# apple/ml-gmpi

Measured on AMD Instinct MI355X. Metric: Mpix*planes/s, higher is better.
Workload: dtype f32; 1 GPU; FFHQ1024-shaped: 1024x1024, 96 planes, batch 4 views, bf16 storage; views_per_gpu=4, views_total=4, H=1024, W=1024, planes=96, variant=auto, strict_order=False, outputs=rgb+depth, parallelism=views sharded x1, poses=truncated-gaussian draw (seed 3) on every rank

## Files before the change

ml-gmpi_amd/csrc/render_band.hip:

```cpp
#include "gmpi_device.hpp"

#include <algorithm>
#include <cstdlib>
#include <type_traits>


namespace gmpi {
namespace band {

constexpr int kNT = 1024;
constexpr int SBW = 64, SBH = 8;
constexpr float kBoxEps = 1.0f / 64;
constexpr int kWindowCols16 = 2, kWindowCols32 = 2, kWindowCols32Deep = 2, kDeepPlanes = 128;
constexpr int kViewRotation = 1;
constexpr int kRunPieces = 2;
constexpr int kTicketTail = 16;
constexpr float kCoordLimit = 16384.0f;

typedef uint32_t u32x4 __attribute__((ext_vector_type(4)));
template <int V> using ic = std::integral_constant<int, V>;

template <int D0, int STEP>
__device__ __forceinline__ void dma16x2(uint32_t voff, uint32_t soff1, const u32x4& rsrc, uint32_t lds_dst, uint64_t m0, uint64_t m1);

#ifndef GMPI_BAND_PPT16
#define GMPI_BAND_PPT16 2
#endif
#ifndef GMPI_BAND_PPT32
#define GMPI_BAND_PPT32 2
#endif
template <typename TexT> struct Geo {
    static constexpr int kES = static_cast<int>(sizeof(TexT));
    static constexpr int NSB = kES == 2 ? 4 : 2;
    static constexpr int PPT = kES == 2 ? GMPI_BAND_PPT16 : GMPI_BAND_PPT32;
    static constexpr int WPS = SBH / PPT;
    static constexpr int kSubLanes = 64 * WPS;
    static constexpr int kThreads = NSB * kSubLanes;
    static constexpr int kWavesPerSimd = kThreads / 128;
    static_assert(kThreads <= kNT && SBH % PPT == 0, "waves");
    static constexpr int kTPI = 16 / kES;
    static constexpr int kCols = kES == 2 ? 10 : 20;
    static constexpr int kLineBytes = kCols * 16;
    static constexpr int kRowBytes = 4 * kLineBytes;
    static constexpr int kIPR = 4 * kCols;
    static constexpr int kMaxRows = 15;
    static constexpr int kCapItems = kMaxRows * kIPR;
    static constexpr int kSubBytes = kCapItems * 16;
    static constexpr int kBufBytes = NSB * kSubBytes;
    static constexpr int kRPP = kSubLanes / kIPR;
    static constexpr int kPassItems = kRPP * kIPR;
    static constexpr int kNP = (kMaxRows + kRPP - 1) / kRPP;
    static_assert(kNP == 3 || kNP == 5, "passes");
    static constexpr int kOffBytes = kThreads * 4;
    static constexpr int kLdsBytes = kOffBytes + 2 * kBufBytes;
};
static_assert(Geo<bf16_t>::kLdsBytes * 2 <= 160 * 1024 && Geo<f16_t>::kLdsBytes * 2 <= 160 * 1024 && Geo<float>::kLdsBytes * 2 <= 160 * 1024, "2 workgroups per CU");

__device__ __forceinline__ void dma16(uint32_t voff, uint32_t soff, const u32x4& rsrc, uint32_t lds_dst, uint64_t mask) {
    uint64_t save;
    asm volatile("s_mov_b64 %0, exec\n\ts_mov_b64 exec, %4\n\ts_mov_b32 m0, %3\n\ts_nop 0\n\tbuffer_load_dwordx4 %1, %2, %5 offen lds\n\ts_mov_b64 exec, %0"
                 : "=&s"(save) : "v"(voff), "s"(rsrc), "s"(lds_dst), "s"(mask), "s"(soff) : "memory");
}
template <int D0, int STEP>
__device__ __forceinline__ void dma16x3(uint32_t voff, uint32_t soff1, uint32_t soff2, const u32x4& rsrc, uint32_t lds_dst, uint64_t m0, uint64_t m1, uint64_t m2) {
    uint64_t save;
    asm volatile("s_mov_b64 %0, exec\n\t"
                 "s_mov_b64 exec, %4\n\ts_add_i32 m0, %3, %9\n\ts_nop 0\n\tbuffer_load_dwordx4 %1, %2, 0 offen lds\n\t"
                 "s_mov_b64 exec, %5\n\ts_add_i32 m0, %3, %10\n\ts_nop 0\n\tbuffer_load_dwordx4 %1, %2, %7 offen lds\n\t"
                 "s_mov_b64 exec, %6\n\ts_add_i32 m0, %3, %11\n\ts_nop 0\n\tbuffer_load_dwordx4 %1, %2, %8 offen lds\n\t"
                 "s_mov_b64 exec, %0"
                 : "=&s"(save) : "v"(voff), "s"(rsrc), "s"(lds_dst), "s"(m0), "s"(m1), "s"(m2), "s"(soff1), "s"(soff2), "i"(D0), "i"(D0 + STEP), "i"(D0 + 2 * STEP)
                 : "memory", "scc");
}
template <int D0, int STEP>
__device__ __forceinline__ void dma16x2(uint32_t voff, uint32_t soff1, const u32x4& rsrc, uint32_t lds_dst, uint64_t m0, uint64_t m1) {
    uint64_t save;
    asm volatile("s_mov_b64 %0, exec\n\t"
                 "s_mov_b64 exec, %4\n\ts_add_i32 m0, %3, %7\n\ts_nop 0\n\tbuffer_load_dwordx4 %1, %2, 0 offen lds\n\t"
                 "s_mov_b64 exec, %5\n\ts_add_i32 m0, %3, %8\n\ts_nop 0\n\tbuffer_load_dwordx4 %1, %2, %6 offen lds\n\t"
                 "s_mov_b64 exec, %0"
                 : "=&s"(save) : "v"(voff), "s"(rsrc), "s"(lds_dst), "s"(m0), "s"(m1), "s"(soff1), "i"(D0), "i"(D0 + STEP)
                 : "memory", "scc");
}
template <int D0, int STEP>
__device__ __forceinline__ void dma16x4(uint32_t voff, uint32_t s1, uint32_t s2, uint32_t s3, const u32x4& rsrc, uint32_t lds_dst, uint64_t m0, uint64_t m1, uint64_t m2, uint64_t m3) {
    uint64_t save;
    asm volatile("s_mov_b64 %0, exec\n\t"
                 "s_mov_b64 exec, %4\n\ts_add_i32 m0, %3, %11\n\ts_nop 0\n\tbuffer_load_dwordx4 %1, %2, 0 offen lds\n\t"
                 "s_mov_b64 exec, %5\n\ts_add_i32 m0, %3, %12\n\ts_nop 0\n\tbuffer_load_dwordx4 %1, %2, %8 offen lds\n\t"
                 "s_mov_b64 exec, %6\n\ts_add_i32 m0, %3, %13\n\ts_nop 0\n\tbuffer_load_dwordx4 %1, %2, %9 offen lds\n\t"
                 "s_mov_b64 exec, %7\n\ts_add_i32 m0, %3, %14\n\ts_nop 0\n\tbuffer_load_dwordx4 %1, %2, %10 offen lds\n\t"
                 "s_mov_b64 exec, %0"
                 : "=&s"(save) : "v"(voff), "s"(rsrc), "s"(lds_dst), "s"(m0), "s"(m1), "s"(m2), "s"(m3), "s"(s1), "s"(s2), "s"(s3),
                   "i"(D0), "i"(D0 + STEP), "i"(D0 + 2 * STEP), "i"(D0 + 3 * STEP)
                 : "memory", "scc");
}
template <int D0, int STEP>
__device__ __forceinline__ void dma16x5(uint32_t voff, uint32_t s1, uint32_t s2, uint32_t s3, uint32_t s4, const u32x4& rsrc, uint32_t lds_dst, uint64_t m0, uint64_t m1, uint64_t m2,
                                        uint64_t m3, uint64_t m4) {
    uint64_t save;
    asm volatile("s_mov_b64 %0, exec\n\t"
                 "s_mov_b64 exec, %4\n\ts_add_i32 m0, %3, %13\n\ts_nop 0\n\tbuffer_load_dwordx4 %1, %2, 0 offen lds\n\t"
                 "s_mov_b64 exec, %5\n\ts_add_i32 m0, %3, %14\n\ts_nop 0\n\tbuffer_load_dwordx4 %1, %2, %9 offen lds\n\t"
                 "s_mov_b64 exec, %6\n\ts_add_i32 m0, %3, %15\n\ts_nop 0\n\tbuffer_load_dwordx4 %1, %2, %10 offen lds\n\t"
                 "s_mov_b64 exec, %7\n\ts_add_i32 m0, %3, %16\n\ts_nop 0\n\tbuffer_load_dwordx4 %1, %2, %11 offen lds\n\t"
                 "s_mov_b64 exec, %8\n\ts_add_i32 m0, %3, %17\n\ts_nop 0\n\tbuffer_load_dwordx4 %1, %2, %12 offen lds\n\t"
                 "s_mov_b64 exec, %0"
                 : "=&s"(save) : "v"(voff), "s"(rsrc), "s"(lds_dst), "s"(m0), "s"(m1), "s"(m2), "s"(m3), "s"(m4), "s"(s1), "s"(s2), "s"(s3), "s"(s4),
                   "i"(D0), "i"(D0 + STEP), "i"(D0 + 2 * STEP), "i"(D0 + 3 * STEP), "i"(D0 + 4 * STEP)
                 : "memory", "scc");
}
__device__ __forceinline__ void wg_barrier() { asm volatile("s_waitcnt vmcnt(0) lgkmcnt(0)\n\ts_barrier" ::: "memory"); }
template <int O> __device__ __forceinline__ void tap16(uint32_t& t, uint32_t a) {
    asm volatile("ds_read_u16_d16_hi %0, %1 offset:%2" : "=v"(t) : "v"(a), "i"(O));
}
template <int O> __device__ __forceinline__ void tap32x2(uint32_t& t0, uint32_t& t1, uint32_t a) {
    typedef uint32_t u32x2 __attribute__((ext_vector_type(2)));
    u32x2 v;
    asm volatile("ds_read2_b32 %0, %1 offset0:%2 offset1:%3" : "=v"(v) : "v"(a), "i"(O), "i"(O + 1));
    t0 = v.x, t1 = v.y;
}

__device__ __forceinline__ void band_pos(int brem, int bands_x, int bands_y, int wc, int& bxi, int& byi) {
    const int per_window = wc * bands_y;
    const int g = brem / per_window, r = brem - g * per_window;
    const int cols = min(wc, bands_x - g * wc);
    byi = r / cols;
    bxi = g * wc + (r - byi * cols);
}

constexpr int kPlU4 = 2;
__device__ __forceinline__ uint32_t shape_pack(int nq, int rows, int clo, int ncol, int rlo, int nrow, bool inside) {
    return inside ? static_cast<uint32_t>(nq | rows << 5)
                  : static_cast<uint32_t>(nq | rows << 5 | clo << 9 | ncol << 14 | rlo << 19 | nrow << 23) | 0x80000000u;
}
struct Shape { int nq, rows; uint32_t clo, ncol, rlo, nrow; };
__device__ __forceinline__ Shape shape_unpack(uint32_t w) {
    Shape h;
    h.nq = w & 31, h.rows = (w >> 5) & 15;
    const bool padded = (w >> 31) != 0;
    h.clo = padded ? (w >> 9) & 31 : 0u, h.ncol = padded ? (w >> 14) & 31 : static_cast<uint32_t>(h.nq);
    h.rlo = padded ? (w >> 19) & 15 : 0u, h.nrow = padded ? (w >> 23) & 15 : static_cast<uint32_t>(h.rows);
    return h;
}
template <typename TexT, bool AC>
__global__ __launch_bounds__(1024) void band_table_kernel(const KParams p, const int bands_x, const int bands_y, const int n_bands, const float cx, const float cy,
                                                         uint4* __restrict__ recs, uint4* __restrict__ pl, uint32_t* __restrict__ hdr, uint32_t* __restrict__ tickets) {
    using G = Geo<TexT>;
    constexpr int kES = G::kES, kTPI = G::kTPI, kCols = G::kCols, kMaxRows = G::kMaxRows, kRowBytes = G::kRowBytes, kSubBytes = G::kSubBytes;
    constexpr int NSB = G::NSB;
    static_assert(kCols < 32 && kMaxRows < 16, "shape_pack");
    const int band_id = blockIdx.x;
    int n, brem;
    item_to_view(p, band_id, bands_x * bands_y, n, brem);
    int bxi, byi;
    band_pos(brem, bands_x, bands_y, p.band_cols, bxi, byi);
    uint32_t ignore = 0;
    const int m = view_mpi(p, n, ignore);
    const int Ht = p.Ht, Wt = p.Wt, H = p.H, W = p.W;
    const float ex = p.eye_pos[3 * n + 0], ey = p.eye_pos[3 * n + 1], ez = p.eye_pos[3 * n + 2];
    const int64_t HW = static_cast<int64_t>(H) * W;
    const float* __restrict__ rdv = p.ray_dir + static_cast<int64_t>(n) * 3 * HW;
    const TexT* __restrict__ vol = static_cast<const TexT*>(p.rgba) + static_cast<int64_t>(m) * p.s_mpi;
    const int sx0 = min(bxi * (NSB * SBW), W - 1), sy0 = byi * SBH;
    const int by0p = min(sy0, H - 1), by1p = min(sy0 + SBH - 1, H - 1);
    bool unfit = false;
    for (int i = threadIdx.x; i < p.D * NSB; i += blockDim.x) {
        const int b = i % NSB, k = i / NSB;
        const float* __restrict__ dhw = p.dhw + (static_cast<int64_t>(m) * p.D + k) * 3;
        const float d = dhw[0], ph = dhw[1], pw = dhw[2];
        const float zdiff = d - ez;
        const float hw = pw * 0.5f, hh = ph * 0.5f;
        const int bx0p = min(sx0 + b * SBW, W - 1), bx1p = min(sx0 + b * SBW + SBW - 1, W - 1);
        float mnx = __builtin_inff(), mxx = -__builtin_inff(), mny = mnx, mxy = mxx;
        bool finite = true;
        const float rw_a = __builtin_amdgcn_rcpf(hw), rh_a = __builtin_amdgcn_rcpf(hh);
#pragma unroll
        for (int c = 0; c < 4; ++c) {
            const int64_t q = static_cast<int64_t>((c & 2) ? by1p : by0p) * W + ((c & 1) ? bx1p : bx0p);
            float ix, iy, sc;
            const float crz = rdv[2 * HW + q];
            plane_coord_recip<AC>(zdiff, hw, hh, rw_a, rh_a, ex, ey, rdv[q], rdv[HW + q], crz, __builtin_amdgcn_rcpf(crz), cx, cy, ix, iy, sc);
            finite = finite && (fabsf(ix) < kCoordLimit) && (fabsf(iy) < kCoordLimit);
            mnx = fminf(mnx, ix), mxx = fmaxf(mxx, ix), mny = fminf(mny, iy), mxy = fmaxf(mxy, iy);
        }
        int qx0 = 0, by0 = 0, nq = -1, nrows = 0;
        if (finite) {
            const int bx0 = static_cast<int>(floorf(mnx - kBoxEps)), bx1 = static_cast<int>(floorf(mxx + kBoxEps)) + 1;
            by0 = static_cast<int>(floorf(mny - kBoxEps));
            const int by1 = static_cast<int>(floorf(mxy + kBoxEps)) + 1;
            qx0 = bx0 & ~(kTPI - 1);
            nq = (bx1 - qx0) / kTPI + 1;
            nrows = by1 - by0 + 1;
            if (nq > kCols || nrows > kMaxRows) nq = -1;
        }
        uint32_t shape = 0;
        if (nq > 0) {
            const int clo = min(max(-qx0 / kTPI, 0), nq), chi = min(max((Wt - qx0) / kTPI, 0), nq);
            const int rlo = min(max(-by0, 0), nrows), rhi = min(max(Ht - by0, 0), nrows);
            const bool inside = clo == 0 && chi == nq && rlo == 0 && rhi == nrows;
            shape = shape_pack(nq, nrows, clo, chi - clo, rlo, rhi - rlo, inside);
        } else {
            qx0 = 0, by0 = 0;
            unfit = true;
        }
        const uint64_t origin = reinterpret_cast<uint64_t>(vol + (static_cast<int64_t>(k) * p.s_plane + static_cast<int64_t>(by0) * p.s_row + qx0));
        const int gpart = b * kSubBytes - (by0 * kRowBytes + qx0 * kES);
        recs[(static_cast<int64_t>(band_id) * p.D + k) * NSB + b] =
            make_uint4(static_cast<uint32_t>(origin & 0xffffffffu), static_cast<uint32_t>((origin >> 32) & 0xffffu), shape, static_cast<uint32_t>(gpart));
        if (brem == 0 && b == 0) {
            uint4* r = pl + (static_cast<int64_t>(n) * p.D + k) * kPlU4;
            r[0] = make_uint4(__float_as_uint(zdiff), __float_as_uint(hw), __float_as_uint(hh), __float_as_uint(1.0f / hw));
            r[1] = make_uint4(__float_as_uint(1.0f / hh), 0u, 0u, 0u);
        }
    }
    if (blockIdx.x == 0 && threadIdx.x < 8) tickets[threadIdx.x] = 0u;
    const int any_unfit = __syncthreads_or(unfit ? 1 : 0);
    if (threadIdx.x == 0) {
        hdr[band_id] = static_cast<uint32_t>(any_unfit);
        if (any_unfit && p.gate != nullptr) {
            if (p.view_to_mpi == nullptr && p.views_per_mpi > 1) {
                const int first = n / p.views_per_mpi * p.views_per_mpi, size = min(p.views_per_mpi, p.N - first);
                for (int v = 0; v < size; ++v) p.gate[first + v] = p.gate_gen;
            } else {
                p.gate[n] = p.gate_gen;
            }
        }
    }
}

template <typename TexT, bool AC, bool STRICT, bool CHECK>
__global__ __launch_bounds__(Geo<TexT>::kThreads, Geo<TexT>::kWavesPerSimd) void render_band_kernel(const KParams p, const int bands_x, const int bands_y, const int n_bands, const float cx, const float cy,
                                                         const uint4* __restrict__ recs, const uint4* __restrict__ pl, const uint32_t* __restrict__ hdr, uint32_t* __restrict__ tickets) {
    using G = Geo<TexT>;
    constexpr int kES = G::kES, kTPI = G::kTPI, kCols = G::kCols, kNP = G::kNP;
    constexpr int NSB = G::NSB, PPT = G::PPT, WPS = G::WPS, kSubLanes = G::kSubLanes;
    constexpr int kLineBytes = G::kLineBytes, kRowBytes = G::kRowBytes, kSubBytes = G::kSubBytes, kBufBytes = G::kBufBytes;
    constexpr int kRPP = G::kRPP, kPassItems = G::kPassItems;
    constexpr bool BF = kES == 2;
    constexpr bool F16 = std::is_same<TexT, f16_t>::value;

    __shared__ __attribute__((aligned(16))) unsigned char smem[G::kLdsBytes];
    typedef __attribute__((address_space(3))) unsigned char lds_byte;
    const uint32_t tile_base = static_cast<uint32_t>(reinterpret_cast<uintptr_t>((lds_byte*)smem));

    const int group_items = bands_x * bands_y * (p.view_to_mpi == nullptr ? p.views_per_mpi : 1);
    int band_id;
    {
        const int per_xcd = (group_items + 7) / 8, n_groups = (n_bands + group_items - 1) / group_items, static_blocks = per_xcd * 8 * n_groups;
        const int T = min(p.band_tail, per_xcd);
        const int jb = static_cast<int>(blockIdx.x) / 8, x = static_cast<int>(blockIdx.x) % 8;
        const bool ticketed = T > 0 && (static_cast<int>(blockIdx.x) >= static_blocks || (jb / per_xcd == n_groups - 1 && jb % per_xcd >= per_xcd - T));
        if (!ticketed) {
            band_id = blockIdx.x < static_cast<unsigned>(static_blocks) ? xcd_item_per_group(blockIdx.x, group_items, n_bands, p.band_rot, p.band_split) : n_bands;
        } else {
            int* word = reinterpret_cast<int*>(smem + 2 * kBufBytes);
            if (threadIdx.x == 0) {
                int got = n_bands;
                for (int i = 0; i < 8; ++i) {
                    const int q = (x + i) % 8;
                    const int t = static_cast<int>(atomicAdd(tickets + q, 1u));
                    if (t < T) {
                        got = xcd_item_per_group(q + 8 * ((n_groups - 1) * per_xcd + per_xcd - T + t), group_items, n_bands, p.band_rot, p.band_split);
                        break;
                    }
                }
                *word = got;
            }
            __syncthreads();
            band_id = __builtin_amdgcn_readfirstlane(*word);
            __syncthreads();
        }
    }
// ... 30 lines not shown
    const int64_t s_chan = p.s_chan, s_row = p.s_row;

    check_camera_behind(p, vw, brem == 0 && tid == 0);

    const int px = bxi * (NSB * SBW) + sb * SBW + lane;
    const int py0 = byi * SBH + wj;
    const int pxc = min(px, W - 1);
    float rx[PPT], ry[PPT], rz[PPT], rcp_rz[PPT];
    Accum A[PPT];
#pragma unroll
    for (int q = 0; q < PPT; ++q) {
        const int64_t pix = static_cast<int64_t>(min(py0 + WPS * q, H - 1)) * W + pxc;
        rx[q] = rdv[pix], ry[q] = rdv[HW + pix], rz[q] = rdv[2 * HW + pix];
        rcp_rz[q] = 1.0f / rz[q];
    }
    auto ray_dot = [&](int q) { return gmpi::ray_dot(vw, rx[q], ry[q], rz[q]); };

    auto loader_pos = [&](int& l_col, int& l_line, int& l_row, bool& l_on) {
        const int t = fresh_tid() & (kSubLanes - 1);
        l_line = t / kCols, l_col = t - l_line * kCols, l_row = l_line >> 2, l_on = t < kPassItems;
    };
    {
        int l_col, l_line, l_row;
        bool l_on;
        loader_pos(l_col, l_line, l_row, l_on);
        reinterpret_cast<uint32_t*>(smem + 2 * kBufBytes)[tid] = static_cast<uint32_t>(l_row * s_row + (l_line & 3) * s_chan + kTPI * l_col) * static_cast<uint32_t>(kES);
    }
    const uint32_t pass_off = static_cast<uint32_t>(kRPP * s_row) * static_cast<uint32_t>(kES), pass_off2 = 2 * pass_off;
    const uint32_t pass_off3 = 3 * pass_off, pass_off4 = 4 * pass_off;
    const uint32_t sub_base = tile_base + static_cast<uint32_t>(sb * kSubBytes);
    const uint32_t wave_dst = sub_base + static_cast<uint32_t>(wj) * 1024u;

#ifdef GMPI_TUNE
    const bool abl_noload = (p.flags & (1u << 16)) != 0, abl_nocomp = (p.flags & (1u << 17)) != 0, abl_noissue = (p.flags & (1u << 18)) != 0;
    const bool abl_nobar = (p.flags & (1u << 20)) != 0, abl_norec = (p.flags & (1u << 21)) != 0;
#else
    constexpr bool abl_noload = false, abl_nocomp = false, abl_noissue = false, abl_nobar = false, abl_norec = false;
#endif

#ifdef GMPI_PROF
    uint32_t prof_acc[8] = {0, 0, 0, 0, 0, 0, 0, 0};
    uint64_t prof_last, prof_start;
    asm volatile("s_memtime %0\n\ts_waitcnt lgkmcnt(0)" : "=s"(prof_start));
    prof_last = prof_start;
#define GMPI_STAMP(i) do { uint64_t now_; asm volatile("s_memtime %0\n\ts_waitcnt lgkmcnt(0)" : "=s"(now_)); prof_acc[i] += static_cast<uint32_t>(now_ - prof_last); prof_last = now_; } while (0)
#else
#define GMPI_STAMP(i) do { } while (0)
#endif

    const uint4* __restrict__ myrec = recs + (static_cast<int64_t>(band_id) * D * NSB + sb);
    const uint4* __restrict__ mypl = pl + static_cast<int64_t>(n) * D * kPlU4;
    constexpr int kRecStep = NSB;

    if (hdr[band_id] != 0) {
#pragma unroll
        for (int q = 0; q < PPT; ++q) {
            const float dot = ray_dot(q);
            for (int t = 0; t < D; ++t) {
                uint32_t gbad = 0;
                gather_plane<TexT, AC, STRICT>(p, vw, vol, t, dhw[3 * t] - ez, dhw[3 * t + 1], dhw[3 * t + 2], rx[q], ry[q], rz[q], dot, std::bool_constant<CHECK>{}, gbad, A[q]);
                if (check_range && __any(gbad != 0)) bad_w |= GMPI_STATUS_RGBA_RANGE;
            }
        }
    } else {
        float dots[PPT];
#pragma unroll
        for (int q = 0; q < PPT; ++q) dots[q] = STRICT ? ray_dot(q) : 0.0f;
        uint64_t m_cur[kNP];
        int dims_cur = 0;
        bool three = false;
        int np_cur = kNP - 1;
#pragma unroll
        for (int r = 0; r < kNP; ++r) m_cur[r] = 0;

        auto issue = [&](const uint4& rl, uint32_t g_off, auto ub) {
            constexpr int U = decltype(ub)::value;
            const int dims = static_cast<int>(rl.z);
            const u32x4 rsrc = {static_cast<uint32_t>(__builtin_amdgcn_readfirstlane(static_cast<int>(rl.x))),
                                static_cast<uint32_t>(__builtin_amdgcn_readfirstlane(static_cast<int>(rl.y))), 0x80000000u, 0x00020000u};
            if (dims >= 0) {
                if (dims != dims_cur) {
                    const int nq = dims & 31, rows = dims >> 5;
                    dims_cur = dims;
                    three = rows > (kNP - 1) * kRPP;
                    np_cur = max((rows + kRPP - 1) / kRPP, 3);
                    int l_col, l_line, l_row;
                    bool l_on;
                    loader_pos(l_col, l_line, l_row, l_on);
#pragma unroll
                    for (int r = 0; r < kNP; ++r) {
                        m_cur[r] = __ballot(l_on && l_col < nq && l_row + r * kRPP < rows);
                        if (abl_noload) m_cur[r] = 0;
                    }
                }
                if constexpr (kNP == 3) {
                    if (three) dma16x3<U * kBufBytes, kPassItems * 16>(g_off, pass_off, pass_off2, rsrc, wave_dst, m_cur[0], m_cur[1], m_cur[2]);
                    else dma16x2<U * kBufBytes, kPassItems * 16>(g_off, pass_off, rsrc, wave_dst, m_cur[0], m_cur[1]);
                } else {
                    if (np_cur == 5) dma16x5<U * kBufBytes, kPassItems * 16>(g_off, pass_off, pass_off2, pass_off3, pass_off4, rsrc, wave_dst, m_cur[0], m_cur[1], m_cur[2], m_cur[3], m_cur[4]);
                    else if (np_cur == 4) dma16x4<U * kBufBytes, kPassItems * 16>(g_off, pass_off, pass_off2, pass_off3, rsrc, wave_dst, m_cur[0], m_cur[1], m_cur[2], m_cur[3]);
                    else dma16x3<U * kBufBytes, kPassItems * 16>(g_off, pass_off, pass_off2, rsrc, wave_dst, m_cur[0], m_cur[1], m_cur[2]);
                }
            } else {
                const Shape h = shape_unpack(static_cast<uint32_t>(dims));
                const int rows = h.rows;
                const uint32_t clo = h.clo, ncol = h.ncol, llo = 4 * h.rlo, nline = 4 * h.nrow;
                dims_cur = dims;
                three = rows > (kNP - 1) * kRPP;
                const int npk = (rows + kRPP - 1) / kRPP;
                np_cur = max(npk, 3);
                int l_col, l_line, l_row;
                bool l_on;
                loader_pos(l_col, l_line, l_row, l_on);
#pragma unroll
                for (int r = 0; r < kNP; ++r) {
                    m_cur[r] = __ballot(l_on && l_row + r * kRPP < rows);
                    if (abl_noload) m_cur[r] = 0;
                    if (r < npk) {
                        const bool ok = (static_cast<uint32_t>(l_col) - clo < ncol) & (static_cast<uint32_t>(l_line + 4 * r * kRPP) - llo < nline);
                        dma16(ok ? g_off : 0x80000000u, r * pass_off, rsrc, wave_dst + static_cast<uint32_t>(U * kBufBytes + r * (kPassItems * 16)), m_cur[r]);
                    }
                }
            }
        };

        uint32_t chk_acc = 0;
        auto tap_fold8 = [&](const uint32_t (&q)[8]) {
            asm volatile("v_max3_u32 %0, %0, %1, %2\n\tv_max3_u32 %0, %0, %3, %4\n\tv_max3_u32 %0, %0, %5, %6\n\tv_max3_u32 %0, %0, %7, %8"
                         : "+v"(chk_acc) : "v"(q[0]), "v"(q[1]), "v"(q[2]), "v"(q[3]), "v"(q[4]), "v"(q[5]), "v"(q[6]), "v"(q[7]));
        };

        auto tapf = [&](uint32_t t) -> float {
            if constexpr (F16) {
                typedef _Float16 h2_t __attribute__((ext_vector_type(2)));
                return static_cast<float>(__builtin_bit_cast(h2_t, t).y);
            } else {
                return __uint_as_float(t);
            }
        };
        struct Coords { float s, nw, ne, sw, se; uint32_t a_tap; };
        auto coords = [&](int q, const float4& rf, const float2& rg, Coords& c) {
            float ix, iy, fx, fy;
            if (STRICT) {
                float u, v;
                plane_coord<AC>(rf.x, rf.z + rf.z, rf.y + rf.y, ex, ey, rx[q], ry[q], rz[q], cx, cy, ix, iy, c.s, u, v);
                fx = floorf(ix), fy = floorf(iy);
                const float fx1 = fx + 1.0f, fy1 = fy + 1.0f;
                const float wx1 = ix - fx, wx0 = fx1 - ix, wy1 = iy - fy, wy0 = fy1 - iy;
                c.nw = wx0 * wy0, c.ne = wx1 * wy0, c.sw = wx0 * wy1, c.se = wx1 * wy1;
            } else {
                plane_coord_recip<AC>(rf.x, rf.y, rf.z, rf.w, rg.x, ex, ey, rx[q], ry[q], rz[q], rcp_rz[q], cx, cy, ix, iy, c.s);
                fx = floorf(ix), fy = floorf(iy);
                const float wx1 = ix - fx, wy1 = iy - fy;
                const float wx0 = 1.0f - wx1, wy0 = 1.0f - wy1;
                c.nw = wx0 * wy0, c.ne = wx1 * wy0, c.sw = wx0 * wy1, c.se = wx1 * wy1;
            }
            const float af = __builtin_fmaf(fy, static_cast<float>(kRowBytes), __builtin_fmaf(fx, static_cast<float>(kES), rg.y));
            c.a_tap = static_cast<uint32_t>(static_cast<int32_t>(af));
        };
        auto taps = [&](auto hb, uint32_t a_tap, uint32_t (&q)[8]) {
            constexpr int C0 = 2 * decltype(hb)::value;
            if constexpr (BF) {
                asm volatile("ds_read_u16_d16_hi %0, %8 offset:%9\n\tds_read_u16_d16_hi %1, %8 offset:%10\n\tds_read_u16_d16_hi %2, %8 offset:%11\n\tds_read_u16_d16_hi %3, %8 offset:%12\n\t"
                             "ds_read_u16_d16_hi %4, %8 offset:%13\n\tds_read_u16_d16_hi %5, %8 offset:%14\n\tds_read_u16_d16_hi %6, %8 offset:%15\n\tds_read_u16_d16_hi %7, %8 offset:%16\n\t"
                             "s_waitcnt lgkmcnt(0)"
                             : "=&v"(q[0]), "=&v"(q[1]), "=&v"(q[2]), "=&v"(q[3]), "=&v"(q[4]), "=&v"(q[5]), "=&v"(q[6]), "=&v"(q[7])
                             : "v"(a_tap), "i"(C0 * kLineBytes), "i"(C0 * kLineBytes + 2), "i"(C0 * kLineBytes + kRowBytes), "i"(C0 * kLineBytes + kRowBytes + 2),
                               "i"((C0 + 1) * kLineBytes), "i"((C0 + 1) * kLineBytes + 2), "i"((C0 + 1) * kLineBytes + kRowBytes), "i"((C0 + 1) * kLineBytes + kRowBytes + 2));
            } else {
                typedef uint32_t u32x2 __attribute__((ext_vector_type(2)));
                u32x2 v0, v1, v2, v3;
// ... 11 lines not shown
                         "ds_read_u16_d16_hi %4, %8 offset:%13\n\tds_read_u16_d16_hi %5, %8 offset:%14\n\tds_read_u16_d16_hi %6, %8 offset:%15\n\tds_read_u16_d16_hi %7, %8 offset:%16"
                         : "=&v"(q[0]), "=&v"(q[1]), "=&v"(q[2]), "=&v"(q[3]), "=&v"(q[4]), "=&v"(q[5]), "=&v"(q[6]), "=&v"(q[7])
                         : "v"(a_tap), "i"(C0 * kLineBytes), "i"(C0 * kLineBytes + 2), "i"(C0 * kLineBytes + kRowBytes), "i"(C0 * kLineBytes + kRowBytes + 2),
                           "i"((C0 + 1) * kLineBytes), "i"((C0 + 1) * kLineBytes + 2), "i"((C0 + 1) * kLineBytes + kRowBytes), "i"((C0 + 1) * kLineBytes + kRowBytes + 2));
        };
        auto taps_land = [&](auto nb, uint32_t (&q)[8]) {
            constexpr int N = decltype(nb)::value;
            asm volatile("s_waitcnt lgkmcnt(%8)" : "+v"(q[0]), "+v"(q[1]), "+v"(q[2]), "+v"(q[3]), "+v"(q[4]), "+v"(q[5]), "+v"(q[6]), "+v"(q[7]) : "i"(N));
        };
        typedef uint32_t u32x2_t __attribute__((ext_vector_type(2)));
        auto taps32_issue = [&](auto hb, uint32_t a_tap, uint32_t a_bot, u32x2_t (&v)[4]) {
            constexpr int C0 = 2 * decltype(hb)::value;
            asm volatile("ds_read2_b32 %0, %4 offset0:%6 offset1:%7\n\tds_read2_b32 %1, %5 offset0:%6 offset1:%7\n\t"
                         "ds_read2_b32 %2, %4 offset0:%8 offset1:%9\n\tds_read2_b32 %3, %5 offset0:%8 offset1:%9"
                         : "=&v"(v[0]), "=&v"(v[1]), "=&v"(v[2]), "=&v"(v[3])
                         : "v"(a_tap), "v"(a_bot), "i"(C0 * (kLineBytes / 4)), "i"(C0 * (kLineBytes / 4) + 1), "i"((C0 + 1) * (kLineBytes / 4)), "i"((C0 + 1) * (kLineBytes / 4) + 1));
        };
        auto taps32_land = [&](auto nb, u32x2_t (&v)[4]) {
            constexpr int N = decltype(nb)::value;
            asm volatile("s_waitcnt lgkmcnt(%4)" : "+v"(v[0]), "+v"(v[1]), "+v"(v[2]), "+v"(v[3]) : "i"(N));
        };
        auto pixel = [&](int q, const float4& rf, const float2& rg) {
            Coords c;
            coords(q, rf, rg, c);
            Footprint f;
            f.nw = c.nw, f.ne = c.ne, f.sw = c.sw, f.se = c.se;
            uint32_t t[8];
            float smp[4];
            taps(ic<0>{}, c.a_tap, t);
            if (check_range) tap_fold8(t);
            smp[0] = bilerp<STRICT>(tapf(t[0]), tapf(t[1]), tapf(t[2]), tapf(t[3]), f);
            smp[1] = bilerp<STRICT>(tapf(t[4]), tapf(t[5]), tapf(t[6]), tapf(t[7]), f);
            taps(ic<1>{}, c.a_tap, t);
            if (check_range) tap_fold8(t);
            smp[2] = bilerp<STRICT>(tapf(t[0]), tapf(t[1]), tapf(t[2]), tapf(t[3]), f);
            smp[3] = bilerp<STRICT>(tapf(t[4]), tapf(t[5]), tapf(t[6]), tapf(t[7]), f);
            blend<STRICT>(A[q], smp[0], smp[1], smp[2], smp[3], c.s, dots[q]);
        };


        uint4 Ln, Fc;
        uint32_t rhh_c, gp_c;
        uint32_t g_off = 0;
#ifdef GMPI_PROF
        constexpr bool piped = false, pipedG = false;
#else
        constexpr bool piped = BF && !STRICT && PPT == 2 && kNP == 3;
        constexpr bool pipedG = !STRICT && !piped;
#endif
        auto stage = [&](int tt, auto ub) {
            constexpr int U = decltype(ub)::value;
            if (!abl_nobar) wg_barrier();
            GMPI_STAMP(0);
            if (tt + 1 < D && !abl_noissue) issue(Ln, g_off, ic<1 - U>{});
            GMPI_STAMP(3);
            const float4 rf = make_float4(__uint_as_float(Fc.x), __uint_as_float(Fc.y), __uint_as_float(Fc.z), __uint_as_float(Fc.w));
            const float2 rg = make_float2(__uint_as_float(rhh_c), static_cast<float>(static_cast<int>(gp_c) + static_cast<int>(tile_base) + U * kBufBytes));
            if constexpr (piped) {
                if (!abl_nocomp) {
                    uint32_t ta[8], tb[8];
                    Coords p0, p1;
                    Footprint f;
                    float smp[4];
                    coords(0, rf, rg, p0);
                    taps_issue(ic<0>{}, p0.a_tap, ta);
                    taps_issue(ic<1>{}, p0.a_tap, tb);
                    coords(1, rf, rg, p1);
                    asm volatile("" : "+v"(p1.s), "+v"(p1.nw), "+v"(p1.ne), "+v"(p1.sw), "+v"(p1.se), "+v"(p1.a_tap));
                    taps_land(ic<8>{}, ta);
                    if (check_range) tap_fold8(ta);
                    f.nw = p0.nw, f.ne = p0.ne, f.sw = p0.sw, f.se = p0.se;
                    smp[0] = bilerp<false>(tapf(ta[0]), tapf(ta[1]), tapf(ta[2]), tapf(ta[3]), f);
                    smp[1] = bilerp<false>(tapf(ta[4]), tapf(ta[5]), tapf(ta[6]), tapf(ta[7]), f);
                    asm volatile("" : "+v"(smp[0]), "+v"(smp[1]));
                    taps_issue(ic<0>{}, p1.a_tap, ta);
                    taps_land(ic<8>{}, tb);
                    if (check_range) tap_fold8(tb);
                    smp[2] = bilerp<false>(tapf(tb[0]), tapf(tb[1]), tapf(tb[2]), tapf(tb[3]), f);
                    smp[3] = bilerp<false>(tapf(tb[4]), tapf(tb[5]), tapf(tb[6]), tapf(tb[7]), f);
                    blend<false>(A[0], smp[0], smp[1], smp[2], smp[3], p0.s, dots[0]);
                    asm volatile("" : "+v"(A[0].T), "+v"(A[0].r), "+v"(A[0].g), "+v"(A[0].b), "+v"(A[0].z));
                    taps_issue(ic<1>{}, p1.a_tap, tb);
                    taps_land(ic<8>{}, ta);
                    if (check_range) tap_fold8(ta);
                    f.nw = p1.nw, f.ne = p1.ne, f.sw = p1.sw, f.se = p1.se;
                    smp[0] = bilerp<false>(tapf(ta[0]), tapf(ta[1]), tapf(ta[2]), tapf(ta[3]), f);
                    smp[1] = bilerp<false>(tapf(ta[4]), tapf(ta[5]), tapf(ta[6]), tapf(ta[7]), f);
                    asm volatile("" : "+v"(smp[0]), "+v"(smp[1]));
                    taps_land(ic<0>{}, tb);
                    if (check_range) tap_fold8(tb);
                    smp[2] = bilerp<false>(tapf(tb[0]), tapf(tb[1]), tapf(tb[2]), tapf(tb[3]), f);
                    smp[3] = bilerp<false>(tapf(tb[4]), tapf(tb[5]), tapf(tb[6]), tapf(tb[7]), f);
                    blend<false>(A[1], smp[0], smp[1], smp[2], smp[3], p1.s, dots[1]);
                }
            } else if constexpr (pipedG) {
                constexpr int NB = BF ? 8 : 4;
                if (!abl_nocomp) {
                    uint32_t ta[8], tb[8];
                    u32x2_t va[4], vb[4];
                    Coords pc, pn;
                    Footprint f;
                    float smp[4];
                    auto issueA = [&](const Coords& c) {
                        if constexpr (BF) taps_issue(ic<0>{}, c.a_tap, ta);
                        else taps32_issue(ic<0>{}, c.a_tap, c.a_tap + kRowBytes, va);
                    };
                    auto issueB = [&](const Coords& c) {
// ... 26 lines not shown
                            smp[2] = bilerp<false>(__uint_as_float(vb[0].x), __uint_as_float(vb[0].y), __uint_as_float(vb[1].x), __uint_as_float(vb[1].y), f);
                            smp[3] = bilerp<false>(__uint_as_float(vb[2].x), __uint_as_float(vb[2].y), __uint_as_float(vb[3].x), __uint_as_float(vb[3].y), f);
                        }
                    };
                    auto px_step = [&](auto qc) {
                        constexpr int Q = decltype(qc)::value;
                        constexpr bool more = Q + 1 < PPT;
                        if constexpr (more) {
                            coords(Q + 1, rf, rg, pn);
                            asm volatile("" : "+v"(pn.s), "+v"(pn.nw), "+v"(pn.ne), "+v"(pn.sw), "+v"(pn.se), "+v"(pn.a_tap));
                        }
                        f.nw = pc.nw, f.ne = pc.ne, f.sw = pc.sw, f.se = pc.se;
                        landA(ic<NB>{});
                        if constexpr (more) issueA(pn);
                        landB(ic<(more ? NB : 0)>{});
                        blend<false>(A[Q], smp[0], smp[1], smp[2], smp[3], pc.s, dots[Q]);
                        if constexpr (more) {
                            asm volatile("" : "+v"(A[Q].T), "+v"(A[Q].r), "+v"(A[Q].g), "+v"(A[Q].b), "+v"(A[Q].z));
                            issueB(pn);
                            pc = pn;
                        }
                    };
                    coords(0, rf, rg, pc);
                    issueA(pc);
                    issueB(pc);
                    px_step(ic<0>{});
                    if constexpr (PPT > 1) px_step(ic<1>{});
                    if constexpr (PPT > 2) px_step(ic<2>{});
                    if constexpr (PPT > 3) px_step(ic<3>{});
                    static_assert(PPT <= 4, "pixel slots");
                }
            } else {
                GMPI_STAMP(2);
                if (!abl_nocomp) {
#pragma unroll
                    for (int q = 0; q < PPT; ++q) {
                        pixel(q, rf, rg);
                        GMPI_STAMP(5 + q);
                    }
                }
            }
            if (!abl_norec) {
                gp_c = Ln.w;
                Ln = myrec[static_cast<int64_t>(tt + 2) * kRecStep];
                Fc = mypl[(tt + 1) * kPlU4], rhh_c = mypl[(tt + 1) * kPlU4 + 1].x;
            }
            static_assert(PPT <= 4 && kNP <= 5, "pixel slots / check passes");
        };
#pragma unroll
        for (int q = 0; q < PPT; ++q)
            asm volatile("" : "+v"(rx[q]), "+v"(ry[q]), "+v"(rz[q]), "+v"(rcp_rz[q]), "+v"(A[q].T), "+v"(A[q].r), "+v"(A[q].g), "+v"(A[q].b), "+v"(A[q].z));
        __syncthreads();
        g_off = reinterpret_cast<const uint32_t*>(smem + 2 * kBufBytes)[fresh_tid()];
        issue(myrec[0], g_off, ic<0>{});
        Fc = mypl[0], rhh_c = mypl[1].x, gp_c = myrec[0].w, Ln = myrec[kRecStep];
        for (int t = 0; t < D; t += 2) {
            stage(t, ic<0>{});
            if (t + 1 < D) stage(t + 1, ic<1>{});
        }
        if (check_range) {
            constexpr uint32_t kOne = F16 ? 0x3c00u : BF ? 0x3f80u : 0x3f800000u, kNegZero = BF ? 0x8000u : 0x80000000u;
            const uint32_t mx = BF ? chk_acc >> 16 : chk_acc;
#ifdef GMPI_TUNE
            if (p.status != nullptr && mx > kOne) { atomicMax(p.status + 1, mx); atomicMax(p.status + 2, static_cast<uint32_t>(band_id)); atomicMax(p.status + 3, static_cast<uint32_t>(tid)); }
#endif
            if (__any(mx > kOne)) {
                if (__any(mx > kOne && mx != kNegZero)) bad_w |= GMPI_STATUS_RGBA_RANGE;
                else {
                    int l_col, l_line, l_row;
                    bool l_on;
                    loader_pos(l_col, l_line, l_row, l_on);
                    const uint32_t g0 = reinterpret_cast<const uint32_t*>(smem + 2 * kBufBytes)[fresh_tid()];
                    bool lane_bad = false;
                    for (int t = 0; t < D; ++t) {
                        const uint4 rl = myrec[static_cast<int64_t>(t) * kRecStep];
                        const Shape h = shape_unpack(rl.z);
                        const int nq = h.nq;
                        const uint32_t clo = h.clo, ncol = h.ncol, llo = 4 * h.rlo, nline = 4 * h.nrow;
                        const unsigned char* org = reinterpret_cast<const unsigned char*>((static_cast<uint64_t>(rl.y) << 32) | rl.x);
                        for (int r = 0; r < kNP; ++r) {
                            const bool in = l_on && l_col < nq && (static_cast<uint32_t>(l_col) - clo < ncol) && (static_cast<uint32_t>(l_line + 4 * r * kRPP) - llo < nline);
                            if (!in) continue;
                            const uint4 q = *reinterpret_cast<const uint4*>(org + g0 + static_cast<uint32_t>(r) * pass_off);
                            const uint32_t d[4] = {q.x, q.y, q.z, q.w};
#pragma unroll
                            for (int c = 0; c < 4; ++c) {
                                if (BF) lane_bad |= !((d[c] & 0xffffu) <= kOne || (d[c] & 0xffffu) == kNegZero) || !((d[c] >> 16) <= kOne || (d[c] >> 16) == kNegZero);
                                else lane_bad |= !(d[c] <= kOne || d[c] == kNegZero);
                            }
                        }
                    }
                    if (__any(lane_bad)) bad_w |= GMPI_STATUS_RGBA_RANGE;
                }
            }
        }
    }

    uint32_t bad = bad_w;
    const LastPlane lp = last_plane(p, vw);
    const int px_e = bxi * (NSB * SBW) + sb * SBW + (fresh_tid() & 63);
#pragma unroll
    for (int q = 0; q < PPT; ++q) {
        const int py = byi * SBH + wj + WPS * q;
        if (leaves_last_plane<AC>(vw, lp, rx[q], ry[q], rz[q])) bad |= GMPI_STATUS_OUT_OF_LAST_PLANE;
        store_pixel<STRICT>(p, n, HW, static_cast<int64_t>(py) * W + px_e, A[q], ray_dot(q), px_e < W && py < H);
    }
    report_status(p.status, bad);
#ifdef GMPI_TUNE
    if (stamp && threadIdx.x == 0) {
        uint64_t stamp_end;
        uint32_t xcc;
        asm volatile("s_memrealtime %0\n\ts_getreg_b32 %1, hwreg(HW_REG_XCC_ID)\n\ts_waitcnt lgkmcnt(0)" : "=s"(stamp_end), "=s"(xcc));
        p.status[64 + 3 * blockIdx.x] = static_cast<uint32_t>(stamp_start), p.status[65 + 3 * blockIdx.x] = static_cast<uint32_t>(stamp_end), p.status[66 + 3 * blockIdx.x] = xcc & 15u;
    }
#endif
#ifdef GMPI_PROF
    if (p.status != nullptr && band_id == 700 && threadIdx.x == 320) {
        uint64_t now_;
        asm volatile("s_memtime %0\n\ts_waitcnt lgkmcnt(0)" : "=s"(now_));
        for (int i = 0; i < 8; ++i) p.status[8 + i] = prof_acc[i];
        p.status[16] = static_cast<uint32_t>(now_ - prof_start);
    }
#endif
}

static int nsb_of(int dtype) { return dtype != 0 ? Geo<bf16_t>::NSB : Geo<float>::NSB; }
static void band_grid(const KParams& p, int nsb, int& bands_x, int& bands_y, int& n_bands) {
    bands_x = (p.W + nsb * SBW - 1) / (nsb * SBW), bands_y = (p.H + SBH - 1) / SBH;
    n_bands = bands_x * bands_y * p.N;
}
static uint64_t align256(uint64_t v) { return (v + 255) / 256 * 256; }
static uint64_t ws_hdr_bytes(int n_bands, int n_views) { return align256((static_cast<uint64_t>(n_bands) + n_views + 8) * 4); }
static uint64_t ws_pl_bytes(const KParams& p) { return align256((static_cast<uint64_t>(p.N) * p.D + 2) * kPlU4 * 16); }
static uint64_t ws_bytes(const KParams& p, int nsb) {
    int bx, by, nb;
    band_grid(p, nsb, bx, by, nb);
    return ws_hdr_bytes(nb, p.N) + ws_pl_bytes(p) + (static_cast<uint64_t>(nb) * p.D + 2) * nsb * 16;
}

template <typename TexT>
static hipError_t launch_t(const KParams& p, hipStream_t stream) {
    constexpr int NSB = Geo<TexT>::NSB;
    int bands_x, bands_y, n_bands;
    band_grid(p, NSB, bands_x, bands_y, n_bands);
    const int group_items = bands_x * bands_y * (p.view_to_mpi == nullptr ? p.views_per_mpi : 1);
    const int tail = std::min(p.band_tail, (group_items + 7) / 8);
// ... 67 lines not shown
```

Baseline: 528,100 Mpix*planes/s.

## Stage fitting prefix planes via LDS DMA, gather only the unfit tail

Per band, the first plane whose footprint does not fit the LDS window is recorded in a shared atomicMin and packed into the record's high bits. The render kernel now runs the staged DMA pipeline for planes before that index and falls back to the per-pixel gather path only for the remaining planes, instead of sending the whole band to gather when any plane is unfit. A whole band is still handed over when the unfit count exceeds a fraction of planes set by a density knob. The DMA helpers are unified into the 3- and 5-pass variants with early exit on empty exec masks. This adds some setup bookkeeping and a barrier per tail plane.

New measurement: 533,300 Mpix*planes/s, median of 6. No clear change (+1.0%).

```diff
diff --git a/ml-gmpi_amd/csrc/render_band.hip b/ml-gmpi_amd/csrc/render_band.hip
--- a/ml-gmpi_amd/csrc/render_band.hip
+++ b/ml-gmpi_amd/csrc/render_band.hip
@@ -16,12 +16,15 @@
 constexpr int kRunPieces = 2;
 constexpr int kTicketTail = 16;
 constexpr float kCoordLimit = 16384.0f;
+#ifndef GMPI_BAND_GATHER_DEN16
+#define GMPI_BAND_GATHER_DEN16 4
+#endif
+#ifndef GMPI_BAND_GATHER_DEN32
+#define GMPI_BAND_GATHER_DEN32 4
+#endif
 
 typedef uint32_t u32x4 __attribute__((ext_vector_type(4)));
 template <int V> using ic = std::integral_constant<int, V>;
-
-template <int D0, int STEP>
-__device__ __forceinline__ void dma16x2(uint32_t voff, uint32_t soff1, const u32x4& rsrc, uint32_t lds_dst, uint64_t m0, uint64_t m1);
 
 #ifndef GMPI_BAND_PPT16
 #define GMPI_BAND_PPT16 2
@@ -65,34 +68,11 @@
 __device__ __forceinline__ void dma16x3(uint32_t voff, uint32_t soff1, uint32_t soff2, const u32x4& rsrc, uint32_t lds_dst, uint64_t m0, uint64_t m1, uint64_t m2) {
     uint64_t save;
     asm volatile("s_mov_b64 %0, exec\n\t"
-                 "s_mov_b64 exec, %4\n\ts_add_i32 m0, %3, %9\n\ts_nop 0\n\tbuffer_load_dwordx4 %1, %2, 0 offen lds\n\t"
-                 "s_mov_b64 exec, %5\n\ts_add_i32 m0, %3, %10\n\ts_nop 0\n\tbuffer_load_dwordx4 %1, %2, %7 offen lds\n\t"
-                 "s_mov_b64 exec, %6\n\ts_add_i32 m0, %3, %11\n\ts_nop 0\n\tbuffer_load_dwordx4 %1, %2, %8 offen lds\n\t"
-                 "s_mov_b64 exec, %0"
+                 "s_mov_b64 exec, %4\n\ts_cbranch_execz 1f\n\ts_add_i32 m0, %3, %9\n\ts_nop 0\n\tbuffer_load_dwordx4 %1, %2, 0 offen lds\n\t"
+                 "s_mov_b64 exec, %5\n\ts_cbranch_execz 1f\n\ts_add_i32 m0, %3, %10\n\ts_nop 0\n\tbuffer_load_dwordx4 %1, %2, %7 offen lds\n\t"
+                 "s_mov_b64 exec, %6\n\ts_cbranch_execz 1f\n\ts_add_i32 m0, %3, %11\n\ts_nop 0\n\tbuffer_load_dwordx4 %1, %2, %8 offen lds\n"
+                 "1:\n\ts_mov_b64 exec, %0"
                  : "=&s"(save) : "v"(voff), "s"(rsrc), "s"(lds_dst), "s"(m0), "s"(m1), "s"(m2), "s"(soff1), "s"(soff2), "i"(D0), "i"(D0 + STEP), "i"(D0 + 2 * STEP)
-                 : "memory", "scc");
-}
-template <int D0, int STEP>
-__device__ __forceinline__ void dma16x2(uint32_t voff, uint32_t soff1, const u32x4& rsrc, uint32_t lds_dst, uint64_t m0, uint64_t m1) {
-    uint64_t save;
-    asm volatile("s_mov_b64 %0, exec\n\t"
-                 "s_mov_b64 exec, %4\n\ts_add_i32 m0, %3, %7\n\ts_nop 0\n\tbuffer_load_dwordx4 %1, %2, 0 offen lds\n\t"
-                 "s_mov_b64 exec, %5\n\ts_add_i32 m0, %3, %8\n\ts_nop 0\n\tbuffer_load_dwordx4 %1, %2, %6 offen lds\n\t"
-                 "s_mov_b64 exec, %0"
-                 : "=&s"(save) : "v"(voff), "s"(rsrc), "s"(lds_dst), "s"(m0), "s"(m1), "s"(soff1), "i"(D0), "i"(D0 + STEP)
-                 : "memory", "scc");
-}
-template <int D0, int STEP>
-__device__ __forceinline__ void dma16x4(uint32_t voff, uint32_t s1, uint32_t s2, uint32_t s3, const u32x4& rsrc, uint32_t lds_dst, uint64_t m0, uint64_t m1, uint64_t m2, uint64_t m3) {
-    uint64_t save;
-    asm volatile("s_mov_b64 %0, exec\n\t"
-                 "s_mov_b64 exec, %4\n\ts_add_i32 m0, %3, %11\n\ts_nop 0\n\tbuffer_load_dwordx4 %1, %2, 0 offen lds\n\t"
-                 "s_mov_b64 exec, %5\n\ts_add_i32 m0, %3, %12\n\ts_nop 0\n\tbuffer_load_dwordx4 %1, %2, %8 offen lds\n\t"
-                 "s_mov_b64 exec, %6\n\ts_add_i32 m0, %3, %13\n\ts_nop 0\n\tbuffer_load_dwordx4 %1, %2, %9 offen lds\n\t"
-                 "s_mov_b64 exec, %7\n\ts_add_i32 m0, %3, %14\n\ts_nop 0\n\tbuffer_load_dwordx4 %1, %2, %10 offen lds\n\t"
-                 "s_mov_b64 exec, %0"
-                 : "=&s"(save) : "v"(voff), "s"(rsrc), "s"(lds_dst), "s"(m0), "s"(m1), "s"(m2), "s"(m3), "s"(s1), "s"(s2), "s"(s3),
-                   "i"(D0), "i"(D0 + STEP), "i"(D0 + 2 * STEP), "i"(D0 + 3 * STEP)
                  : "memory", "scc");
 }
 template <int D0, int STEP>
@@ -100,12 +80,12 @@
                                         uint64_t m3, uint64_t m4) {
     uint64_t save;
     asm volatile("s_mov_b64 %0, exec\n\t"
-                 "s_mov_b64 exec, %4\n\ts_add_i32 m0, %3, %13\n\ts_nop 0\n\tbuffer_load_dwordx4 %1, %2, 0 offen lds\n\t"
-                 "s_mov_b64 exec, %5\n\ts_add_i32 m0, %3, %14\n\ts_nop 0\n\tbuffer_load_dwordx4 %1, %2, %9 offen lds\n\t"
-                 "s_mov_b64 exec, %6\n\ts_add_i32 m0, %3, %15\n\ts_nop 0\n\tbuffer_load_dwordx4 %1, %2, %10 offen lds\n\t"
-                 "s_mov_b64 exec, %7\n\ts_add_i32 m0, %3, %16\n\ts_nop 0\n\tbuffer_load_dwordx4 %1, %2, %11 offen lds\n\t"
-                 "s_mov_b64 exec, %8\n\ts_add_i32 m0, %3, %17\n\ts_nop 0\n\tbuffer_load_dwordx4 %1, %2, %12 offen lds\n\t"
-                 "s_mov_b64 exec, %0"
+                 "s_mov_b64 exec, %4\n\ts_cbranch_execz 1f\n\ts_add_i32 m0, %3, %13\n\ts_nop 0\n\tbuffer_load_dwordx4 %1, %2, 0 offen lds\n\t"
+                 "s_mov_b64 exec, %5\n\ts_cbranch_execz 1f\n\ts_add_i32 m0, %3, %14\n\ts_nop 0\n\tbuffer_load_dwordx4 %1, %2, %9 offen lds\n\t"
+                 "s_mov_b64 exec, %6\n\ts_cbranch_execz 1f\n\ts_add_i32 m0, %3, %15\n\ts_nop 0\n\tbuffer_load_dwordx4 %1, %2, %10 offen lds\n\t"
+                 "s_mov_b64 exec, %7\n\ts_cbranch_execz 1f\n\ts_add_i32 m0, %3, %16\n\ts_nop 0\n\tbuffer_load_dwordx4 %1, %2, %11 offen lds\n\t"
+                 "s_mov_b64 exec, %8\n\ts_cbranch_execz 1f\n\ts_add_i32 m0, %3, %17\n\ts_nop 0\n\tbuffer_load_dwordx4 %1, %2, %12 offen lds\n"
+                 "1:\n\ts_mov_b64 exec, %0"
                  : "=&s"(save) : "v"(voff), "s"(rsrc), "s"(lds_dst), "s"(m0), "s"(m1), "s"(m2), "s"(m3), "s"(m4), "s"(s1), "s"(s2), "s"(s3), "s"(s4),
                    "i"(D0), "i"(D0 + STEP), "i"(D0 + 2 * STEP), "i"(D0 + 3 * STEP), "i"(D0 + 4 * STEP)
                  : "memory", "scc");
@@ -164,7 +144,9 @@
     const TexT* __restrict__ vol = static_cast<const TexT*>(p.rgba) + static_cast<int64_t>(m) * p.s_mpi;
     const int sx0 = min(bxi * (NSB * SBW), W - 1), sy0 = byi * SBH;
     const int by0p = min(sy0, H - 1), by1p = min(sy0 + SBH - 1, H - 1);
-    bool unfit = false;
+    __shared__ int first_unfit[NSB];
+    if (threadIdx.x < NSB) first_unfit[threadIdx.x] = p.D;
+    __syncthreads();
     for (int i = threadIdx.x; i < p.D * NSB; i += blockDim.x) {
         const int b = i % NSB, k = i / NSB;
         const float* __restrict__ dhw = p.dhw + (static_cast<int64_t>(m) * p.D + k) * 3;
@@ -202,7 +184,7 @@
             shape = shape_pack(nq, nrows, clo, chi - clo, rlo, rhi - rlo, inside);
         } else {
             qx0 = 0, by0 = 0;
-            unfit = true;
+            atomicMin(&first_unfit[b], k);
         }
         const uint64_t origin = reinterpret_cast<uint64_t>(vol + (static_cast<int64_t>(k) * p.s_plane + static_cast<int64_t>(by0) * p.s_row + qx0));
         const int gpart = b * kSubBytes - (by0 * kRowBytes + qx0 * kES);
@@ -215,10 +197,24 @@
         }
     }
     if (blockIdx.x == 0 && threadIdx.x < 8) tickets[threadIdx.x] = 0u;
-    const int any_unfit = __syncthreads_or(unfit ? 1 : 0);
+    __syncthreads();
+    int unfit = 0;
+    for (int i = threadIdx.x; i < p.D * NSB; i += blockDim.x) {
+        const int b = i % NSB, k = i / NSB;
+        unfit += k >= first_unfit[b] ? 1 : 0;
+        if (k == 0) {
+            reinterpret_cast<uint32_t*>(recs + static_cast<int64_t>(band_id) * p.D * NSB + b)[1] |= static_cast<uint32_t>(min(first_unfit[b], 0xffff)) << 16;
+        }
+    }
+    int n_unfit = 0;
+    for (int j = 0; j * static_cast<int>(blockDim.x) < p.D * NSB; ++j) n_unfit += __syncthreads_count(unfit > j);
+    const bool shared_mpi = p.view_to_mpi == nullptr && p.views_per_mpi > 1;
+    constexpr int den = kES == 2 ? GMPI_BAND_GATHER_DEN16 : GMPI_BAND_GATHER_DEN32;
+    const int limit = shared_mpi || den == 0 ? 0 : p.D * NSB / max(den, 1);
+    const bool hand_over = n_unfit > limit;
     if (threadIdx.x == 0) {
-        hdr[band_id] = static_cast<uint32_t>(any_unfit);
-        if (any_unfit && p.gate != nullptr) {
+        hdr[band_id] = hand_over ? 1u : 0u;
+        if (hand_over && p.gate != nullptr) {
             if (p.view_to_mpi == nullptr && p.views_per_mpi > 1) {
                 const int first = n / p.views_per_mpi * p.views_per_mpi, size = min(p.views_per_mpi, p.N - first);
                 for (int v = 0; v < size; ++v) p.gate[first + v] = p.gate_gen;
@@ -355,24 +351,13 @@
     const uint4* __restrict__ mypl = pl + static_cast<int64_t>(n) * D * kPlU4;
     constexpr int kRecStep = NSB;
 
-    if (hdr[band_id] != 0) {
-#pragma unroll
-        for (int q = 0; q < PPT; ++q) {
-            const float dot = ray_dot(q);
-            for (int t = 0; t < D; ++t) {
-                uint32_t gbad = 0;
-                gather_plane<TexT, AC, STRICT>(p, vw, vol, t, dhw[3 * t] - ez, dhw[3 * t + 1], dhw[3 * t + 2], rx[q], ry[q], rz[q], dot, std::bool_constant<CHECK>{}, gbad, A[q]);
-                if (check_range && __any(gbad != 0)) bad_w |= GMPI_STATUS_RGBA_RANGE;
-            }
-        }
-    } else {
+    const int Dh = __builtin_amdgcn_readfirstlane(hdr[band_id] != 0 ? 0 : min(static_cast<int>(myrec[0].y >> 16), D));
+    if (Dh > 0) {
         float dots[PPT];
 #pragma unroll
         for (int q = 0; q < PPT; ++q) dots[q] = STRICT ? ray_dot(q) : 0.0f;
         uint64_t m_cur[kNP];
         int dims_cur = 0;
-        bool three = false;
-        int np_cur = kNP - 1;
 #pragma unroll
         for (int r = 0; r < kNP; ++r) m_cur[r] = 0;
 
@@ -385,8 +370,6 @@
                 if (dims != dims_cur) {
                     const int nq = dims & 31, rows = dims >> 5;
                     dims_cur = dims;
-                    three = rows > (kNP - 1) * kRPP;
-                    np_cur = max((rows + kRPP - 1) / kRPP, 3);
                     int l_col, l_line, l_row;
                     bool l_on;
                     loader_pos(l_col, l_line, l_row, l_on);
@@ -396,22 +379,13 @@
                         if (abl_noload) m_cur[r] = 0;
                     }
                 }
-                if constexpr (kNP == 3) {
-                    if (three) dma16x3<U * kBufBytes, kPassItems * 16>(g_off, pass_off, pass_off2, rsrc, wave_dst, m_cur[0], m_cur[1], m_cur[2]);
-                    else dma16x2<U * kBufBytes, kPassItems * 16>(g_off, pass_off, rsrc, wave_dst, m_cur[0], m_cur[1]);
-                } else {
-                    if (np_cur == 5) dma16x5<U * kBufBytes, kPassItems * 16>(g_off, pass_off, pass_off2, pass_off3, pass_off4, rsrc, wave_dst, m_cur[0], m_cur[1], m_cur[2], m_cur[3], m_cur[4]);
-                    else if (np_cur == 4) dma16x4<U * kBufBytes, kPassItems * 16>(g_off, pass_off, pass_off2, pass_off3, rsrc, wave_dst, m_cur[0], m_cur[1], m_cur[2], m_cur[3]);
-                    else dma16x3<U * kBufBytes, kPassItems * 16>(g_off, pass_off, pass_off2, rsrc, wave_dst, m_cur[0], m_cur[1], m_cur[2]);
-                }
+                if constexpr (kNP == 3) dma16x3<U * kBufBytes, kPassItems * 16>(g_off, pass_off, pass_off2, rsrc, wave_dst, m_cur[0], m_cur[1], m_cur[2]);
+                else dma16x5<U * kBufBytes, kPassItems * 16>(g_off, pass_off, pass_off2, pass_off3, pass_off4, rsrc, wave_dst, m_cur[0], m_cur[1], m_cur[2], m_cur[3], m_cur[4]);
             } else {
                 const Shape h = shape_unpack(static_cast<uint32_t>(dims));
                 const int rows = h.rows;
                 const uint32_t clo = h.clo, ncol = h.ncol, llo = 4 * h.rlo, nline = 4 * h.nrow;
                 dims_cur = dims;
-                three = rows > (kNP - 1) * kRPP;
-                const int npk = (rows + kRPP - 1) / kRPP;
-                np_cur = max(npk, 3);
                 int l_col, l_line, l_row;
                 bool l_on;
                 loader_pos(l_col, l_line, l_row, l_on);
@@ -419,7 +393,7 @@
                 for (int r = 0; r < kNP; ++r) {
                     m_cur[r] = __ballot(l_on && l_row + r * kRPP < rows);
                     if (abl_noload) m_cur[r] = 0;
-                    if (r < npk) {
+                    if (m_cur[r] != 0) {
                         const bool ok = (static_cast<uint32_t>(l_col) - clo < ncol) & (static_cast<uint32_t>(l_line + 4 * r * kRPP) - llo < nline);
                         dma16(ok ? g_off : 0x80000000u, r * pass_off, rsrc, wave_dst + static_cast<uint32_t>(U * kBufBytes + r * (kPassItems * 16)), m_cur[r]);
                     }
@@ -537,7 +511,7 @@
             constexpr int U = decltype(ub)::value;
             if (!abl_nobar) wg_barrier();
             GMPI_STAMP(0);
-            if (tt + 1 < D && !abl_noissue) issue(Ln, g_off, ic<1 - U>{});
+            if (tt + 1 < Dh && !abl_noissue) issue(Ln, g_off, ic<1 - U>{});
             GMPI_STAMP(3);
             const float4 rf = make_float4(__uint_as_float(Fc.x), __uint_as_float(Fc.y), __uint_as_float(Fc.z), __uint_as_float(Fc.w));
             const float2 rg = make_float2(__uint_as_float(rhh_c), static_cast<float>(static_cast<int>(gp_c) + static_cast<int>(tile_base) + U * kBufBytes));
@@ -670,11 +644,15 @@
             asm volatile("" : "+v"(rx[q]), "+v"(ry[q]), "+v"(rz[q]), "+v"(rcp_rz[q]), "+v"(A[q].T), "+v"(A[q].r), "+v"(A[q].g), "+v"(A[q].b), "+v"(A[q].z));
         __syncthreads();
         g_off = reinterpret_cast<const uint32_t*>(smem + 2 * kBufBytes)[fresh_tid()];
-        issue(myrec[0], g_off, ic<0>{});
+        {
+            uint4 r0 = myrec[0];
+            r0.y &= 0xffffu;
+            issue(r0, g_off, ic<0>{});
+        }
         Fc = mypl[0], rhh_c = mypl[1].x, gp_c = myrec[0].w, Ln = myrec[kRecStep];
-        for (int t = 0; t < D; t += 2) {
+        for (int t = 0; t < Dh; t += 2) {
             stage(t, ic<0>{});
-            if (t + 1 < D) stage(t + 1, ic<1>{});
+            if (t + 1 < Dh) stage(t + 1, ic<1>{});
         }
         if (check_range) {
             constexpr uint32_t kOne = F16 ? 0x3c00u : BF ? 0x3f80u : 0x3f800000u, kNegZero = BF ? 0x8000u : 0x80000000u;
@@ -690,12 +668,12 @@
                     loader_pos(l_col, l_line, l_row, l_on);
                     const uint32_t g0 = reinterpret_cast<const uint32_t*>(smem + 2 * kBufBytes)[fresh_tid()];
                     bool lane_bad = false;
-                    for (int t = 0; t < D; ++t) {
+                    for (int t = 0; t < Dh; ++t) {
                         const uint4 rl = myrec[static_cast<int64_t>(t) * kRecStep];
                         const Shape h = shape_unpack(rl.z);
                         const int nq = h.nq;
                         const uint32_t clo = h.clo, ncol = h.ncol, llo = 4 * h.rlo, nline = 4 * h.nrow;
-                        const unsigned char* org = reinterpret_cast<const unsigned char*>((static_cast<uint64_t>(rl.y) << 32) | rl.x);
+                        const unsigned char* org = reinterpret_cast<const unsigned char*>((static_cast<uint64_t>(rl.y & 0xffffu) << 32) | rl.x);
                         for (int r = 0; r < kNP; ++r) {
                             const bool in = l_on && l_col < nq && (static_cast<uint32_t>(l_col) - clo < ncol) && (static_cast<uint32_t>(l_line + 4 * r * kRPP) - llo < nline);
                             if (!in) continue;
@@ -710,6 +688,24 @@
                     }
                     if (__any(lane_bad)) bad_w |= GMPI_STATUS_RGBA_RANGE;
                 }
+            }
+        }
+    }
+
+    if (Dh < D) {
+        const bool in_band = hdr[band_id] == 0;
+        if (in_band && Dh == 0) {
+            if (sb == 0) *reinterpret_cast<uint4*>(smem + 16 * (fresh_tid() & (kSubLanes - 1))) = make_uint4(0u, 0u, 0u, 0u);
+            __syncthreads();
+        }
+#pragma unroll
+        for (int q = 0; q < PPT; ++q) {
+            const float dot = ray_dot(q);
+            for (int t = Dh; t < D; ++t) {
+                if (q == 0 && in_band) wg_barrier();
+                uint32_t gbad = 0;
+                gather_plane<TexT, AC, STRICT>(p, vw, vol, t, dhw[3 * t] - ez, dhw[3 * t + 1], dhw[3 * t + 2], rx[q], ry[q], rz[q], dot, std::bool_constant<CHECK>{}, gbad, A[q]);
+                if (check_range && __any(gbad != 0)) bad_w |= GMPI_STATUS_RGBA_RANGE;
             }
         }
     }
```
